# omerkurt-okt/buck-gnn

Hardware: AMD Instinct MI355X
Metric: graphs/sec (fwd+bwd) 6-layer SAGE h=512, ~5k-node meshes, batch 16, 1/2/4/8 GPU (higher is better)
Workload: dtype f32

## Files before the change

buck-gnn_amd/bgnn/_lib.py:

```python
from __future__ import annotations

import ctypes
import os
import threading

_HERE = os.path.dirname(os.path.abspath(__file__))
LIB_PATH = os.environ.get("BGNN_LIBRARY") or os.path.join(_HERE, "_lib", "libbgnn.so")
ABI_VERSION = 15

_lock = threading.Lock()
_lib = None

c_p = ctypes.c_void_p
c_i32 = ctypes.c_int32
c_i64 = ctypes.c_int64
c_f32 = ctypes.c_float
c_u64 = ctypes.c_uint64
c_sz = ctypes.c_size_t


class CsrStruct(ctypes.Structure):

    _fields_ = [
        ("rowptr", c_p),
        ("col", c_p),
        ("heavy_row", c_p),
        ("heavy_chunk0", c_p),
        ("chunk_heavy", c_p),
        ("n_rows", c_i64),
        ("nnz", c_i64),
        ("n_heavy", c_i32),
        ("n_chunks", c_i32),
        ("chunk", c_i32),
        ("ranges_all", c_i32),
        ("gsrc", c_p),
        ("gmask", c_p),
        ("gcnt", c_p),
        ("grow", c_p),
        ("n_groups", c_i64),
        ("group_rows", c_i32),
        ("_pad2", c_i32),
        ("ranges", c_p),
    ]


SIGNATURES = {
    "bgnn_abi_version": (c_i32, []),
    "bgnn_last_error_string": (ctypes.c_char_p, []),
    "bgnn_store_gather_graph": (c_i32, [c_p, c_i32, c_i64, c_i64, c_i64, c_i64, c_p, c_i64, c_p, c_p, c_p, c_p,
                                        c_p, c_p, c_p, c_p, c_p, c_p, c_p, c_p, c_p]),
    "bgnn_store_gather_rows": (c_i32, [c_p, c_i32, c_i32, c_i64, c_p, c_i64, c_p, c_p]),
    "bgnn_get_tuning": (c_i32, [c_i32]),
    "bgnn_heavy_timing": (c_i32, [c_i32]),
    "bgnn_gemm_w_tile": (c_i32, [c_i64, c_i64, c_i64]),
    "bgnn_gemm_wsplit_bytes": (c_sz, [c_i64, c_i64]),
    "bgnn_gemm_wsplit": (c_i32, [c_p, c_i32, c_i64, c_i64, c_i64, c_i64, c_p, c_i64, c_p, c_i64, c_i32, c_p]),
    "bgnn_gemm_f32_w": (c_i32, [c_i64, c_i64, c_i64, c_p, c_i64, c_p, c_i32, c_p, c_i64, c_p, c_i32, c_p, c_p, c_p,
                                c_p, c_i64, c_f32, c_u64, c_p]),
    "bgnn_heavy_timing_read": (c_i32, [c_i32, c_p, c_p]),
    "bgnn_set_tuning": (c_i32, [c_i32, c_i32]),
    "bgnn_graph_build_ws_bytes": (c_sz, [c_i64, c_i64]),
    "bgnn_graph_build": (c_i32, [c_p, c_i64, c_i64, c_p, c_p, c_p, c_p, c_p, c_p, c_sz, c_p, c_p]),
    "bgnn_index_csr_build": (c_i32, [c_p, c_i64, c_i64, c_p, c_p, c_p, c_sz, c_p, c_p]),
    "bgnn_heavy_plan_ws_bytes": (c_sz, [c_i64]),
    "bgnn_heavy_plan": (c_i32, [c_p, c_i64, c_i64, c_i32, c_p, c_p, c_p, c_p, c_p, c_sz, c_p]),
    "bgnn_spmm_fwd": (c_i32, [ctypes.POINTER(CsrStruct), c_p, c_i64, c_i32, c_i32, c_p, c_i64, c_p, c_p, c_p]),
    "bgnn_spmm_bwd": (c_i32, [ctypes.POINTER(CsrStruct), c_p, c_p, c_p, c_i64, c_i32, c_i32, c_p, c_i64, c_p, c_p,
                              c_i32, c_p]),
    "bgnn_heavy_ranges_bytes": (c_sz, [c_i32]),
    "bgnn_heavy_ranges": (c_i32, [ctypes.POINTER(CsrStruct), c_p, c_p]),
    "bgnn_range_partial_bytes": (c_sz, [c_i64, c_i32]),
    "bgnn_range_sums_finish": (c_i32, [c_p, c_i64, c_i32, ctypes.POINTER(CsrStruct), c_i32, c_p, c_i64, c_p, c_p,
                                       c_p]),
    "bgnn_bn_slots": (c_i32, [c_i64, c_i32]),
    "bgnn_bn_stats": (c_i32, [c_p, c_i64, c_i32, c_p, c_p]),
    "bgnn_bn_apply": (c_i32, [c_p, c_i64, c_i32, c_p, c_p, c_p, c_p]),
    "bgnn_bn_bwd_stats": (c_i32, [c_p, c_p, c_p, c_p, c_i64, c_i32, c_p, c_p]),
    "bgnn_bn_bwd_dx": (c_i32, [c_p, c_p, c_p, c_p, c_p, c_p, c_i64, c_i32, c_p, c_p]),
    "bgnn_spmm_bwd_add": (c_i32, [ctypes.POINTER(CsrStruct), c_p, c_p, c_p, c_i64, c_i32, c_i32, c_p, c_i64, c_p,
                                  c_i64, c_p, c_p, c_p]),
    "bgnn_spmm_bwd_max": (c_i32, [ctypes.POINTER(CsrStruct), c_p, c_p, c_i64, c_p, c_i64, c_i32, c_p, c_p, c_i64, c_p,
                                  c_i64, c_p, c_p, c_p]),
    "bgnn_spmm_max_arg_bytes": (c_sz, [c_i64, c_i32, c_i32]),
    "bgnn_sage_fwd_slots": (c_i32, [ctypes.POINTER(CsrStruct)]),
    "bgnn_group_plan": (c_i32, [c_p, c_p, c_i64, c_i32, c_i32, c_p, c_i64, c_p, c_p, c_p, c_p]),
    "bgnn_store_gather_groups": (c_i32, [c_p, c_i32, c_i32, c_i64, c_i64, c_i64, c_i64] + [c_p] * 14),
    "bgnn_sage_fwd": (c_i32, [ctypes.POINTER(CsrStruct), c_p, c_i64, c_p, c_i64, c_p, c_i32, c_i32, c_p, c_p, c_p,
                              c_p, c_p, c_i64, c_p]),
    "bgnn_bn_finalize": (c_i32, [c_p, c_i32, c_i32, c_i64, c_p, c_p, c_f32, c_f32, c_p, c_p, c_p, c_p, c_p, c_p,
                                 c_p]),
    "bgnn_bn_finalize_shifted": (c_i32, [c_p, c_i32, c_i32, c_i64, c_p, c_p, c_p, c_f32, c_f32, c_p, c_p, c_p, c_p, c_p, c_p,
                                 c_p]),
    "bgnn_bn_eval_coeffs": (c_i32, [c_i32, c_p, c_p, c_f32, c_p, c_p, c_p, c_p, c_p]),
    "bgnn_sage_apply": (c_i32, [c_p, c_p, c_p, c_p, c_i32, c_f32, c_u64, c_i64, c_i32, c_p, c_p, c_p, c_p, c_p]),
    "bgnn_sage_infer_bf16": (c_i32, [ctypes.POINTER(CsrStruct), c_p, c_i64, c_p, c_p, c_p, c_p, c_i64, c_i32, c_i32,
                                     c_p, c_i64, c_i32, c_p, c_p]),
    "bgnn_spmm_fwd_bf16": (c_i32, [ctypes.POINTER(CsrStruct), c_p, c_i64, c_i32, c_i32, c_p, c_i64, c_i32, c_p, c_p]),
    "bgnn_spmm_bwd_bf16": (c_i32, [ctypes.POINTER(CsrStruct), c_p, c_p, c_i64, c_i32, c_i32, c_p, c_i64, c_i32, c_p,
                                   c_p]),
# ... 108 lines not shown
```

buck-gnn_amd/bgnn/fused.py:

```python
from __future__ import annotations

import torch

from . import _lib
from .graph import Graph, _stream, require_cuda

GEMM_BACKEND = "hip"

PLANE_TILE = 128
Z_PLANES = False
DZ_PLANES = False
DGRAD_WT = True
FOLD_WEIGHTS_TORCH = False
DGRAD_DROPADD = True

BF16_PREP = True
ABSMAX_ITEMS = True
PERSISTENT_WPACK = True
MAX_MERGED = True
WSPLIT = True

TIMERS = None
TIMER_EVENT = None


class _timed:
    __slots__ = ("name", "ev")

    def __init__(self, name):
        self.name = name
        self.ev = None

    def __enter__(self):
        if TIMERS is not None:
            mk = TIMER_EVENT or (lambda: torch.cuda.Event(enable_timing=True))
            self.ev = (mk(), mk())
            self.ev[0].record()
        return self

    def __exit__(self, *exc):
        if self.ev is not None:
            self.ev[1].record()
            TIMERS.setdefault(self.name, []).append(self.ev)
        return False


class Planes:
    __slots__ = ("t",)

    def __init__(self, t: torch.Tensor):
        if t.dim() != 3 or not t.is_contiguous():
            raise ValueError("Planes: need a contiguous [P, rows, blk] tensor")
        self.t = t
# ... 478 lines not shown
        full = torch.empty(N + R, H, dtype=torch.float32, device=dev)
        x_next = full[:N]
        rp = torch.empty(_lib.query("bgnn_range_partial_bytes", N, H) // 4, dtype=torch.float32, device=dev)
        _lib.call("bgnn_sage_apply", o.data_ptr(), _ptr(scale), _ptr(shift), x_prev.data_ptr(), int(cfg.skip),
                  float(cfg.p), cfg.seed, N, H, x_next.data_ptr(), next_amax.data_ptr(), graph.fwd.ranges.data_ptr(),
                  rp.data_ptr(), s)
        _lib.call("bgnn_range_sums_finish", rp.data_ptr(), N, H, graph.fwd.ref(), 0, full[N:].data_ptr(), H,
                  next_amax.data_ptr(), rng.out_amax.data_ptr(), s)
        rng.holder.append(full)
        return x_next, (scale, shift, mean, invstd)
    x_next = torch.empty(N, H, dtype=torch.float32, device=dev)
    _lib.call("bgnn_sage_apply", o.data_ptr(), _ptr(scale), _ptr(shift), x_prev.data_ptr(), int(cfg.skip),
              float(cfg.p), cfg.seed, N, H, x_next.data_ptr(), next_amax.data_ptr(), None, None, s)
    return x_next, (scale, shift, mean, invstd)


def _glue_bwd_stats(g, o, scale, shift, mean, invstd, cfg: LayerConfig, g_rows=None):
    if not cfg.bn:
        return None, None, None, None
    N, H = o.shape
    dev = o.device
    s = _stream()
    rs = _lib.query("bgnn_rows_slots", N)
    part2 = torch.empty(rs, 2, H, dtype=torch.float32, device=dev)
    _lib.call("bgnn_sage_bwd_stats", g.data_ptr(), _ptr(g_rows), o.data_ptr(), scale.data_ptr(), shift.data_ptr(),
              mean.data_ptr(), invstd.data_ptr(), float(cfg.p), cfg.seed, N, H, part2.data_ptr(), s)
    sums = torch.empty(2, H, dtype=torch.float32, device=dev)
    _lib.call("bgnn_reduce_partials", part2.data_ptr(), rs, H, sums[0].data_ptr(), sums[1].data_ptr(), 0, s)
    dbeta, dgamma = sums[0], sums[1]
    if cfg.training:
        return dgamma, dbeta, sums[0], sums[1]
    z = torch.zeros(H, dtype=torch.float32, device=dev)
    return dgamma, dbeta, z, z


class SageLayerFn(torch.autograd.Function):

    @staticmethod
    def forward(ctx, x_prev, x_amax, w_l, b_l, w_r, gamma, beta, running_mean, running_var, graph: Graph,
                cfg: LayerConfig, amax=None, w_in=None, b_in=None, wprep=None, pool=None):
        dev = x_prev.device
        x_prev = x_prev.contiguous()
        H = w_l.size(0)
        N = x_prev.size(0)
        if isinstance(wprep, WPrep):
            wcat, wcat_t_pre, img_f, img_d = wprep.wcat, wprep.wcat_t, wprep, wprep
        elif wprep is not None:
            (wcat, wcat_t_pre), img_f, img_d = wprep, None, None
        else:
            wcat, wcat_t_pre, img_f, img_d = torch.cat([w_l, w_r], 0).contiguous(), None, None, None
        img_f = img_f if (img_f is not None and img_f.img_f is not None) else None
        img_d = img_d if (img_d is not None and img_d.img_d is not None) else None
        if amax is None:
            amax = torch.zeros(3, dtype=torch.float32, device=dev)
        w_amax, next_amax, dz_amax = amax[0:1], amax[1:2], amax[2:3]
        folded = w_in is not None
        if folded:
            if cfg.skip:
                raise ValueError("sage_layer: a folded input transform needs a layer without skip")
            if FOLD_WEIGHTS_TORCH:
                wf = torch.mm(wcat, w_in)
                bf = torch.mv(wcat, b_in)
            else:
                fs = cfg.famax
                fa = (fs[0:1], fs[1:2], fs[2:3]) if fs is not None else (None, None, None)
                if fs is not None:
                    absmax(wcat, fa[0], accumulate=True)
                    absmax(w_in, fa[1], accumulate=True)
                    absmax(b_in.view(1, -1), fa[2], accumulate=True)
                wf = gemm(wcat, w_in.contiguous(), trans_a=False, trans_b=False, a_amax=fa[0], b_amax=fa[1])
                bf = gemm(wcat, b_in.contiguous().view(H, 1), trans_a=False, trans_b=False, a_amax=fa[0],
                          b_amax=fa[2]).view(-1)
            absmax(wf, w_amax, accumulate=True)
            wmat = wf
        else:
            if wprep is None:
                absmax(wcat, w_amax, accumulate=True)
            wmat, bf = wcat, None
        if x_amax is None:
            x_amax = absmax(x_prev)
        planes = Z_PLANES and H % PLANE_TILE == 0 and not folded
        rng = cfg.rng
        x_full = rng.x_full if (rng is not None and rng.x_full is not None and not folded and not planes) else None
        if x_full is not None and x_full.data_ptr() != x_prev.data_ptr():
            raise RuntimeError("sage_layer: RangeRows.x_full must start at x_prev")
        xa, a_amax_g = (x_full, rng.x_amax) if x_full is not None else (x_prev, x_amax)
        M = xa.size(0)
        with _timed("gemm_fwd_fold" if folded else "gemm_fwd"):
            if planes:
                z = torch.empty(2, N, H, dtype=torch.float32, device=dev)
                gemm(x_prev, wmat, trans_a=False, trans_b=True, out=Planes(z), a_amax=x_amax, b_amax=w_amax)
                zl, zr, ldz = z[0], z[1], H
            elif (img_f is not None and not folded
                  and _lib.query("bgnn_gemm_w_tile", M, 2 * H, H) == img_f.bn_f):
                z = torch.empty(M, 2 * H, dtype=torch.float32, device=dev)
                _lib.call("bgnn_gemm_f32_w", M, 2 * H, H, xa.data_ptr(), xa.stride(0), img_f.img_f.data_ptr(),
                          img_f.bn_f, z.data_ptr(), 2 * H, None, 0, a_amax_g.data_ptr(), w_amax.data_ptr(), None, None,
                          0, 0.0, 0, _stream())
                zl, zr, ldz = z, z[:, H:], 2 * H
            else:
                z = gemm(xa, wmat, trans_a=False, trans_b=True, bias=bf, a_amax=a_amax_g, b_amax=w_amax)
                zl, zr, ldz = z, z[:, H:], 2 * H
        hagg = z[N:] if x_full is not None else None
        o = torch.empty(N, H, dtype=torch.float32, device=dev)
        nrm = torch.empty(N, dtype=torch.float32, device=dev)
        slots = _lib.query("bgnn_sage_fwd_slots", graph.fwd.ref())
        bn_part = torch.empty(slots, 2, H, dtype=torch.float32, device=dev)
        part = (torch.empty(graph.fwd.plan.n_chunks * H, dtype=torch.float32, device=dev)
                if graph.fwd.plan.n_chunks else None)
        s = _stream()
        with _timed("sage_fwd"):
            _lib.call("bgnn_sage_fwd", graph.fwd.ref(), zl.data_ptr(), ldz, zr.data_ptr(), ldz, b_l.data_ptr(), H,
                      cfg.reduce, o.data_ptr(), nrm.data_ptr(), bn_part.data_ptr(), _ptr(part), _ptr(hagg),
                      2 * H if hagg is not None else 0, s)
        del z, zl, zr, hagg
        x_next, (scale, shift, mean, invstd) = _glue_fwd(o, bn_part, slots, x_prev, gamma, beta, running_mean,
                                                         running_var, cfg, next_amax, graph)
        ctx.graph = graph
        ctx.cfg = cfg
        ctx.folded = folded
        ctx.wcat_t = wcat_t_pre
        ctx.img_d = img_d if not folded else None
        ctx.set_materialize_grads(False)
        ctx.fold = (w_in, b_in, wf) if folded else None
        ctx.save_for_backward(x_prev, o, nrm, wcat, gamma if gamma is not None else torch.empty(0, device=dev),
                              scale if scale is not None else torch.empty(0, device=dev),
                              shift if shift is not None else torch.empty(0, device=dev),
                              mean if mean is not None else torch.empty(0, device=dev),
                              invstd if invstd is not None else torch.empty(0, device=dev),
                              x_amax, w_amax, dz_amax)
        ctx.mark_non_differentiable(next_amax)
        ctx.pool = pool
        if pool is not None:
            from .ops import spmm_fwd
            pooled, _ = spmm_fwd(pool.fwd, x_next, 1, pool.num_rows)
            return x_next, next_amax, pooled
        return x_next, next_amax

    @staticmethod
    def backward(ctx, g, _g_amax, g_pool=None):
        cfg: LayerConfig = ctx.cfg
        g_rows = None
        if g_pool is not None:
            seg = ctx.pool
            gp = g_pool.contiguous() / seg.fwd.degree().clamp_min(1).to(g_pool.dtype).unsqueeze(1)
            if g is None and not cfg.skip:
                g, g_rows = gp, seg.index
            else:
                gb = gp.index_select(0, seg.index)
                g = gb if g is None else g + gb
        if g is None:
            return (None,) * 16
        x_prev, o, nrm, wcat, gamma, scale, shift, mean, invstd, x_amax, w_amax, dz_amax = ctx.saved_tensors
        graph: Graph = ctx.graph
        g = g.contiguous()
        N, H = o.shape
        planes = DZ_PLANES and H % PLANE_TILE == 0
        dev = o.device
        s = _stream()
        bn = cfg.bn
        dgamma, dbeta, sum_g2, sum_g2xhat = _glue_bwd_stats(g, o, scale, shift, mean, invstd, cfg, g_rows)
        if planes:
            dzt = torch.empty(2, N, H, dtype=torch.float32, device=dev)
            dz, dzl, dh, lddz = Planes(dzt), dzt[0], dzt[1], H
        else:
            dz = torch.empty(N, 2 * H, dtype=torch.float32, device=dev)
            dzl, dh, lddz = dz, dz[:, H:], 2 * H
        dropadd = (cfg.skip and DGRAD_DROPADD and GEMM_BACKEND == "hip" and DGRAD_WT and not planes
                   and H % 4 == 0 and _lib.query("bgnn_get_tuning", 5) == 2)
        gskip = torch.empty(N, H, dtype=torch.float32, device=dev) if (cfg.skip and not dropadd) else None
        rs = _lib.query("bgnn_rows_slots", N)
        part_db = torch.empty(rs, 2, H, dtype=torch.float32, device=dev)
        bw = graph.bwd
        rb = (cfg.rng is not None and cfg.rng.bwd and not planes and bw.ranges is not None)
        rp = (torch.empty(_lib.query("bgnn_range_partial_bytes", N, H) // 4, dtype=torch.float32, device=dev)
              if rb else None)
        _lib.call("bgnn_sage_bwd_rows", g.data_ptr(), _ptr(g_rows), o.data_ptr(), nrm.data_ptr(),
                  _ptr(scale) if bn else None, _ptr(shift) if bn else None,
                  _ptr(gamma) if (bn and gamma.numel()) else None,
                  _ptr(mean) if bn else None, _ptr(invstd) if bn else None, _ptr(sum_g2), _ptr(sum_g2xhat),
                  float(cfg.p), cfg.seed, int(cfg.skip and not dropadd), N, H, dh.data_ptr(), lddz, _ptr(gskip),
                  part_db.data_ptr(), dz_amax.data_ptr(), graph.fwd.rowptr.data_ptr() if ctx.folded else None,
                  (2 if cfg.reduce == 1 else 1) if ctx.folded else 0, _ptr(bw.ranges) if rb else None,
                  graph.fwd.rowptr.data_ptr() if (rb and cfg.reduce == 1) else None, _ptr(rp), s)
        if rb:
            _lib.call("bgnn_range_sums_finish", rp.data_ptr(), N, H, bw.ref(), 1, dzl.data_ptr(), lddz, None,
                      dz_amax.data_ptr(), s)
        db2 = torch.empty(2 if ctx.folded else 1, H, dtype=torch.float32, device=dev)
        _lib.call("bgnn_reduce_partials", part_db.data_ptr(), rs, H, db2[-1].data_ptr(),
                  db2[0].data_ptr() if ctx.folded else None, 0, s)
        db, db_zl = db2[-1], (db2[0] if ctx.folded else None)
        part = torch.empty(bw.plan.n_chunks * H, dtype=torch.float32, device=dev) if bw.plan.n_chunks else None
        with _timed("spmm_bwd"):
            _lib.call("bgnn_spmm_bwd", bw.ref(), graph.perm_t.data_ptr(), graph.fwd.rowptr.data_ptr(),
                      dh.data_ptr(), lddz, H, cfg.reduce, dzl.data_ptr(), lddz, _ptr(part),
                      dz_amax.data_ptr(), int(rb), s)
        has_affine = bn and gamma.numel() > 0
        if ctx.folded:
            w_in, b_in, wf = ctx.fold
            wf_t = wf.t().contiguous() if DGRAD_WT else wf
            with _timed("gemm_dgrad_fold"):
                dx = gemm(dz, wf_t, trans_a=False, trans_b=DGRAD_WT, a_amax=dz_amax, b_amax=w_amax)
            fs = cfg.famax
            fa = (fs[0:1], fs[1:2], fs[2:3], fs[3:4], fs[4:5]) if fs is not None else (None,) * 5
            with _timed("gemm_wgrad_fold"):
                dwf = gemm(dz, x_prev, trans_a=True, trans_b=False, a_amax=dz_amax, b_amax=x_amax,
                           c_amax=fa[3])
            dbf = db2.view(-1)
            if fs is not None:
                absmax(db2, fa[4], accumulate=True)
            if FOLD_WEIGHTS_TORCH:
                dw = torch.addmm(torch.outer(dbf, b_in), dwf, w_in.t())
                dw_in = torch.mm(wcat.t(), dwf)
                db_in = torch.mv(wcat.t(), dbf)
            else:
                dw = gemm(dwf, w_in.contiguous(), trans_a=False, trans_b=True, a_amax=fa[3],
                          b_amax=fa[1])
                dw.add_(torch.outer(dbf, b_in))
                dw_in = gemm(wcat, dwf, trans_a=True, trans_b=False, a_amax=fa[0], b_amax=fa[3])
                db_in = gemm(wcat, dbf.view(-1, 1), trans_a=True, trans_b=False, a_amax=fa[0],
                             b_amax=fa[4]).view(-1)
            return (dx, None, dw[:H], db, dw[H:], dgamma if has_affine else None, dbeta if has_affine else None,
                    None, None, None, None, None, dw_in, db_in, None, None)
        wcat_t = (ctx.wcat_t if ctx.wcat_t is not None else wcat.t().contiguous()) if DGRAD_WT else wcat
        img_d = ctx.img_d if (not planes and DGRAD_WT) else None
        if (img_d is not None and (dropadd or gskip is None)
                and _lib.query("bgnn_gemm_w_tile", N, H, 2 * H) == img_d.bn_d):
            dx = torch.empty(N, H, dtype=torch.float32, device=dev)
            with _timed("gemm_dgrad"):
                _lib.call("bgnn_gemm_f32_w", N, H, 2 * H, dz.data_ptr(), lddz, img_d.img_d.data_ptr(), img_d.bn_d,
                          dx.data_ptr(), H, None, 0, dz_amax.data_ptr(), w_amax.data_ptr(), None,
                          g.data_ptr() if dropadd else None, H, float(cfg.p) if dropadd else 0.0,
                          cfg.seed if dropadd else 0, s)
        elif dropadd:
            dx = torch.empty(N, H, dtype=torch.float32, device=dev)
            M_, K_ = N, 2 * H
            ws_bytes = _lib.query("bgnn_gemm_ws_bytes_ex", M_, H, K_, 0, 1, 0)
            ws = torch.empty(ws_bytes, dtype=torch.uint8, device=dev) if ws_bytes else None
            with _timed("gemm_dgrad"):
                _lib.call("bgnn_gemm_f32_dropadd", 0, 1, M_, H, K_, dz.data_ptr(), lddz, wcat_t.data_ptr(),
                          wcat_t.stride(0), dx.data_ptr(), H, dz_amax.data_ptr(), w_amax.data_ptr(), g.data_ptr(),
                          H, float(cfg.p), cfg.seed, _ptr(ws), ws_bytes, s)
        elif gskip is not None:
            with _timed("gemm_dgrad"):
                dx = gemm(dz, wcat_t, trans_a=False, trans_b=DGRAD_WT, out=gskip, beta=1.0, a_amax=dz_amax,
                          b_amax=w_amax)
        else:
            with _timed("gemm_dgrad"):
                dx = gemm(dz, wcat_t, trans_a=False, trans_b=DGRAD_WT, a_amax=dz_amax, b_amax=w_amax)
        with _timed("gemm_wgrad"):
            dw = gemm(dz, x_prev, trans_a=True, trans_b=False, a_amax=dz_amax, b_amax=x_amax)
        dw_l, dw_r = dw[:H], dw[H:]
        return (dx, None, dw_l, db, dw_r, dgamma if has_affine else None, dbeta if has_affine else None,
                None, None, None, None, None, None, None, None, None)


# ... 436 lines not shown
```

buck-gnn_amd/csrc/spmm.hip:

```cpp
#include <vector>

#include "common.h"
#include "gemm_common.h"
#include "seg_common.h"

namespace bgnn {

enum : int { OP_SUM = 0, OP_MEAN = 1, OP_MAX = 2, OP_MEANT = 3, OP_MAXT = 4 };
enum : int { EPI_PLAIN = 0, EPI_SAGE = 1 };

struct SegArgs {
    const int32_t* rowptr;
    const int32_t* col;
    const int32_t* heavy_row;
    const int32_t* heavy_chunk0;
    const int32_t* chunk_heavy;
    int64_t n_rows;
    int32_t n_heavy, n_chunks, chunk;
    int32_t H;
    int64_t rows_per_block;
    const float* x;     int64_t ldx;
    float* out;         int64_t ldo;
    uint8_t* arg8;
    int32_t* heavy_of;
// ... 5 lines not shown
    const uint8_t* arg8_in;
    const int32_t* heavy_of_in;
    const int32_t* arg_h_in;
    const float* zr;    int64_t ldzr;
    const float* bias;
    float* nrm;
    float* bn_partial;
    int32_t light_slots;
    int32_t nt;
    uint32_t* amax;
    const float* add;
    int64_t ld_add;
    const int32_t* gsrc;
    const uint8_t* gmask;
    const int32_t* gcnt;
    const int32_t* grow;
    int64_t n_groups;
    int32_t group_rows;
    int32_t rev;
    const int32_t* hfirst;
    const float* hagg;
    int64_t ld_hagg;
    int32_t hdone;
    int32_t ranges_all;
};

__device__ __forceinline__ bool range_row(const SegArgs& A, int32_t h) {
    return A.hfirst != nullptr && (A.hagg != nullptr || A.hdone) && A.hfirst[h] >= 0;
}

__device__ __forceinline__ void amax_flush_wave(uint32_t* amax, uint32_t m) {
    if (!amax) return;
    for (int o = 32; o > 0; o >>= 1) m = max(m, (uint32_t)__shfl_xor((int)m, o, kWave));
    if ((threadIdx.x & 63) == 0 && m) atomicMax(amax, m);
}


template <int VEC>
struct Vec {
    float f[VEC];
};

template <int VEC>
__device__ __forceinline__ Vec<VEC> ld(const float* p) {
    Vec<VEC> v;
    if constexpr (VEC == 4) {
        const float4 q = *reinterpret_cast<const float4*>(p);
        v.f[0] = q.x; v.f[1] = q.y; v.f[2] = q.z; v.f[3] = q.w;
    } else {
        v.f[0] = *p;
    }
    return v;
}

template <int VEC>
__device__ __forceinline__ void st(float* p, const Vec<VEC>& v) {
    if constexpr (VEC == 4) {
        *reinterpret_cast<float4*>(p) = make_float4(v.f[0], v.f[1], v.f[2], v.f[3]);
    } else {
        *p = v.f[0];
    }
}

template <int VEC>
__device__ __forceinline__ void ldi(const int32_t* p, int32_t (&o)[VEC]) {
    if constexpr (VEC == 4) {
        const int4 q = *reinterpret_cast<const int4*>(p);
// ... 741 lines not shown
                        *pq = s2;
                    }
                    if (lane == 0) A.nrm[r] = nr;
                }
            } else {
#pragma unroll
                for (int t = 0; t < R; ++t) {
                    const int64_t r = r0 + t;
                    const int32_t rb = __builtin_amdgcn_readlane(rp, t);
                    const int32_t deg = __builtin_amdgcn_readlane(rp, t + 1) - rb;
                    if (t >= rows || deg > chunk) continue;
                    Acc<4, NV, OP> acc;
#pragma unroll
                    for (int v = 0; v < NV; ++v)
#pragma unroll
                        for (int q = 0; q < 4; ++q) acc.a[v][q] = a[t][v][q];
                    store_plain<4, NV, OP>(A, acc, r, deg, cpos, cok, tmax);
                }
            }
        }
    }
    if constexpr (EPI == EPI_PLAIN) amax_flush_wave(A.amax, tmax);

    if constexpr (EPI == EPI_SAGE) {
        __syncthreads();
        float* dst = A.bn_partial + (int64_t)blockIdx.x * 2 * A.H;
        for (int c = threadIdx.x; c < A.H; c += 256) {
            dst[c] = (red[0][0][c] + red[1][0][c]) + (red[2][0][c] + red[3][0][c]);
            dst[A.H + c] = (red[0][1][c] + red[1][1][c]) + (red[2][1][c] + red[3][1][c]);
        }
    }
}

constexpr int kMaxLightBlocks = 1024;

static int g_seg_kernel = 0;
static int g_grp_blocks = 1024;
static int g_seg_blocks = 1024;
static int g_seg_nt = 1;
static int g_seg_u = 0;

struct Geometry {
    int vec, nv, lpr, ctiles;
};

inline int pow2ceil(int x) {
    int p = 1;
    while (p < x) p <<= 1;
    return p;
}

inline Geometry pick_geometry(int H, bool aligned16) {
    Geometry g;
    if (aligned16 && H % 4 == 0) {
        g.vec = 4;
        const int nv4 = H / 4;
        if (nv4 >= 128) { g.lpr = 64; g.nv = 2; }
        else if (nv4 > 64) { g.lpr = 64; g.nv = 2; }
        else { g.lpr = pow2ceil(nv4 < 16 ? 16 : nv4); g.nv = 1; }
        g.ctiles = (H + g.lpr * 4 * g.nv - 1) / (g.lpr * 4 * g.nv);
    } else {
        g.vec = 1;
        g.nv = 1;
        g.lpr = pow2ceil(H < 16 ? 16 : (H > 64 ? 64 : H));
        g.ctiles = (H + g.lpr - 1) / g.lpr;
    }
// ... 163 lines not shown
    A.heavy_chunk0 = c->heavy_chunk0;
    A.chunk_heavy = c->chunk_heavy;
    A.n_rows = c->n_rows;
    A.n_heavy = c->n_heavy;
    A.n_chunks = c->n_chunks;
    A.chunk = c->chunk > 0 ? c->chunk : 0x7fffffff;
    if (c->gsrc && c->gmask && c->gcnt && (c->group_rows == 4 || c->group_rows == 8)) {
        A.gsrc = c->gsrc;
        A.gmask = c->gmask;
        A.gcnt = c->gcnt;
        A.group_rows = c->group_rows;
        A.grow = c->grow;
        A.n_groups = c->grow ? c->n_groups : (c->n_rows + c->group_rows - 1) / c->group_rows;
    }
    if (c->ranges && c->n_heavy > 0) {
        A.hfirst = c->ranges + 2 + 3 * c->n_heavy;
        A.ranges_all = c->ranges_all;
    }
    return A;
}

extern int g_x6_bdma;
extern int g_h3p_nsb;
#ifdef BGNN_H3P_ABLATION
extern int g_h3p_abl;
#endif

}

using namespace bgnn;

extern "C" int bgnn_spmm_fwd(const bgnn_csr_t* csr, const float* x, int64_t ldx, int32_t H, int32_t reduce,
                             float* out, int64_t ldo, void* arg, float* partial, void* stream) {
    BGNN_REQUIRE(csr && csr->rowptr, "spmm_fwd: null csr");
    BGNN_REQUIRE(H > 0 && ldx >= H && ldo >= H, "spmm_fwd: bad H/ld");
    BGNN_REQUIRE(reduce >= 0 && reduce <= 2, "spmm_fwd: bad reduce %d", reduce);
    BGNN_REQUIRE(csr->n_chunks == 0 || partial, "spmm_fwd: partial scratch required for heavy rows");
    SegArgs A = args_from_csr(csr);
    g_heavy_dir = 0;
    A.H = H;
    A.x = x; A.ldx = ldx;
    A.out = out; A.ldo = ldo;
    if (arg) {
        BGNN_REQUIRE(csr->chunk > 0 && csr->chunk < 255,
                     "spmm_fwd(max, arg): the CSR's chunk must be in [1, 254] for the compact argmax (got %d)",
                     csr->chunk);
        const MaxArgLayout L = max_arg_layout(csr->n_rows, H);
        A.arg8 = static_cast<uint8_t*>(arg);
        A.heavy_of = reinterpret_cast<int32_t*>(static_cast<char*>(arg) + L.heavy_of);
        A.arg_h = reinterpret_cast<int32_t*>(static_cast<char*>(arg) + L.arg_h);
    }
    A.partial = partial;
    A.partial_arg = partial ? reinterpret_cast<int32_t*>(partial + (int64_t)csr->n_chunks * H) : nullptr;
    const bool al = aligned16(x) && aligned16(out) && ldx % 4 == 0 && ldo % 4 == 0 &&
                    (!partial || aligned16(partial)) && (!arg || aligned16(arg));
    const Geometry g = pick_geometry(H, al);
    hipStream_t s = as_stream(stream);
    switch (reduce) {
        case BGNN_REDUCE_SUM: return dispatch_plain<OP_SUM>(A, g, s);
        case BGNN_REDUCE_MEAN: return dispatch_plain<OP_MEAN>(A, g, s);
        default: return dispatch_plain<OP_MAX>(A, g, s);
    }
}

static int spmm_bwd_impl(const bgnn_csr_t* csr_t, const int32_t* perm_t, const int32_t* fwd_rowptr,
                         int64_t fwd_rows, const float* g, int64_t ldg, int32_t H, int32_t reduce, const void* arg,
                         const float* addend, int64_t ld_add, float* gx, int64_t ldgx, float* partial, float* amax,
                         int heavy_done, void* stream);

extern "C" int bgnn_spmm_bwd(const bgnn_csr_t* csr_t, const int32_t* perm_t, const int32_t* fwd_rowptr,
                             const float* g, int64_t ldg, int32_t H, int32_t reduce, float* gx, int64_t ldgx,
                             float* partial, float* amax, int32_t heavy_done, void* stream) {
    BGNN_REQUIRE(reduce != BGNN_REDUCE_MAX, "spmm_bwd: max aggregation takes bgnn_spmm_bwd_max");
    BGNN_REQUIRE(!heavy_done || (csr_t && csr_t->ranges), "spmm_bwd: heavy_done needs the CSR's ranges");
    return spmm_bwd_impl(csr_t, perm_t, fwd_rowptr, 0, g, ldg, H, reduce, nullptr, nullptr, 0, gx, ldgx, partial,
                         amax, heavy_done ? 1 : 0, stream);
}

extern "C" int bgnn_spmm_bwd_add(const bgnn_csr_t* csr_t, const int32_t* perm_t, const int32_t* fwd_rowptr,
                                 const float* g, int64_t ldg, int32_t H, int32_t reduce, const float* addend,
                                 int64_t ld_add, float* gx, int64_t ldgx, float* partial, float* amax, void* stream) {
    BGNN_REQUIRE(reduce != BGNN_REDUCE_MAX, "spmm_bwd_add: max aggregation takes bgnn_spmm_bwd_max");
    return spmm_bwd_impl(csr_t, perm_t, fwd_rowptr, 0, g, ldg, H, reduce, nullptr, addend, ld_add, gx, ldgx, partial,
                         amax, 0, stream);
}

// ... 128 lines not shown
                 "sage_fwd: ldzl/ldzr must be >= H and multiples of 4");
    BGNN_REQUIRE(reduce == BGNN_REDUCE_SUM || reduce == BGNN_REDUCE_MEAN, "sage_fwd: reduce must be sum/mean");
    BGNN_REQUIRE(aligned16(zl) && aligned16(zr) && aligned16(o) && aligned16(bias) && aligned16(bn_partial) &&
                     (!partial || aligned16(partial)),
                 "sage_fwd: pointers must be 16-byte aligned");
    BGNN_REQUIRE(csr->n_chunks == 0 || partial, "sage_fwd: partial scratch required for heavy rows");
    SegArgs A = args_from_csr(csr);
    g_heavy_dir = 0;
    A.H = H;
    A.x = zl; A.ldx = ldzl;
    A.zr = zr; A.ldzr = ldzr;
    A.bias = bias;
    A.out = o; A.ldo = H;
    A.nrm = nrm;
    A.bn_partial = bn_partial;
    A.partial = partial;
    if (heavy_agg) {
        BGNN_REQUIRE(csr->ranges && aligned16(heavy_agg) && ld_heavy_agg >= H && ld_heavy_agg % 4 == 0,
                     "sage_fwd: heavy_agg needs the CSR's ranges, 16-B alignment and ld >= H");
        A.hagg = heavy_agg;
        A.ld_hagg = ld_heavy_agg;
    }
    hipStream_t s = as_stream(stream);
    int64_t blocks = 0;
    if (H > 256) {
        return reduce == BGNN_REDUCE_SUM
                   ? launch_all<4, 2, 64, OP_SUM, EPI_SAGE>(A, 1, kMaxLightBlocks, s, &blocks)
                   : launch_all<4, 2, 64, OP_MEAN, EPI_SAGE>(A, 1, kMaxLightBlocks, s, &blocks);
    }
    return reduce == BGNN_REDUCE_SUM ? launch_all<4, 1, 64, OP_SUM, EPI_SAGE>(A, 1, kMaxLightBlocks, s, &blocks)
                                     : launch_all<4, 1, 64, OP_MEAN, EPI_SAGE>(A, 1, kMaxLightBlocks, s, &blocks);
}

extern "C" int bgnn_heavy_timing(int32_t enable) {
    g_heavy_on = enable != 0;
    if (g_heavy_on) g_heavy_used = 0;
    return BGNN_OK;
}

extern "C" int bgnn_heavy_timing_read(int32_t which, float* total_ms, int32_t* count) {
    BGNN_REQUIRE(total_ms && count && (which == 0 || which == 1), "heavy_timing_read: bad args");
    double t = 0.0;
    int32_t n = 0;
    for (size_t i = 0; i < g_heavy_used; ++i) {
        const HeavyEv& e = g_heavy_ev[i];
        if (e.fwd != (which == 0 ? 1 : 0)) continue;
        BGNN_HIP(hipEventSynchronize(e.b));
        float ms = 0.f;
        BGNN_HIP(hipEventElapsedTime(&ms, e.a, e.b));
        t += ms;
        ++n;
    }
    *total_ms = (float)t;
    *count = n;
    return BGNN_OK;
}

extern "C" size_t bgnn_spmm_max_arg_bytes(int64_t rows, int32_t H, int32_t n_heavy) {
    if (rows < 0 || H <= 0 || n_heavy < 0) return 0;
    return (size_t)max_arg_layout(rows, H).arg_h + (size_t)n_heavy * (size_t)H * 4;
}
```

include/bgnn.h:

```cpp
#ifndef BGNN_H
#define BGNN_H

#include <stddef.h>
#include <stdint.h>

#ifdef __cplusplus
extern "C" {
#endif

#define BGNN_ABI_VERSION 15

#define BGNN_OK 0
#define BGNN_E_ARG 1001
#define BGNN_E_WS 1002
#define BGNN_E_UNSUPPORTED 1003

#define BGNN_REDUCE_SUM 0
#define BGNN_REDUCE_MEAN 1
#define BGNN_REDUCE_MAX 2

int bgnn_abi_version(void);
const char* bgnn_last_error_string(void);

#define BGNN_TUNE_SEG_KERNEL 1
#define BGNN_TUNE_SEG_BLOCKS 2
#define BGNN_TUNE_SEG_U 3
#define BGNN_TUNE_SEG_NT 4
#define BGNN_TUNE_GEMM_MODE 5
#define BGNN_TUNE_ROWS_NT 6
#define BGNN_TUNE_GROUP_BLOCKS 7
#define BGNN_TUNE_ROWS_REV 13
#define BGNN_TUNE_GEMM_BDMA 16
int bgnn_heavy_timing(int32_t enable);
int bgnn_heavy_timing_read(int32_t which, float* total_ms, int32_t* count);
int32_t bgnn_get_tuning(int32_t knob);
int bgnn_set_tuning(int32_t knob, int32_t value);

typedef struct bgnn_csr {
    const int32_t* rowptr;
    const int32_t* col;
    const int32_t* heavy_row;
    const int32_t* heavy_chunk0;
    const int32_t* chunk_heavy;
// ... 14 lines not shown
} bgnn_csr_t;

size_t bgnn_graph_build_ws_bytes(int64_t num_edges, int64_t num_nodes);

int bgnn_graph_build(const int64_t* edge_index, int64_t num_edges, int64_t num_nodes,
                     int32_t* rowptr, int32_t* col,
                     int32_t* rowptr_t, int32_t* col_t, int32_t* perm_t,
                     void* ws, size_t ws_bytes, int32_t* dev_status, void* stream);

int bgnn_index_csr_build(const int64_t* index, int64_t n, int64_t num_rows,
                         int32_t* rowptr, int32_t* col,
                         void* ws, size_t ws_bytes, int32_t* dev_status, void* stream);

size_t bgnn_heavy_plan_ws_bytes(int64_t n_rows);
int bgnn_heavy_plan(const int32_t* rowptr, int64_t n_rows, int64_t nnz, int32_t chunk,
                    int32_t* heavy_row, int32_t* heavy_chunk0, int32_t* chunk_heavy,
                    int32_t* dev_counts, void* ws, size_t ws_bytes, void* stream);

size_t bgnn_heavy_ranges_bytes(int32_t n_heavy);
int bgnn_heavy_ranges(const bgnn_csr_t* csr, int32_t* ranges, void* stream);

size_t bgnn_range_partial_bytes(int64_t n_rows, int32_t H);
int bgnn_range_sums_finish(const float* range_partial, int64_t n_rows, int32_t H, const bgnn_csr_t* csr,
                           int32_t mode, float* out, int64_t ldo, const float* amax_floor, float* amax,
                           void* stream);

int bgnn_group_plan(const int32_t* rowptr, const int32_t* col, int64_t n_rows, int32_t chunk,
                    int32_t group_rows, const int32_t* grow, int64_t n_groups,
                    int32_t* gsrc, uint8_t* gmask, int32_t* gcnt, void* stream);

int bgnn_spmm_fwd(const bgnn_csr_t* csr, const float* x, int64_t ldx, int32_t H,
                  int32_t reduce, float* out, int64_t ldo, void* arg,
                  float* partial, void* stream);
size_t bgnn_spmm_max_arg_bytes(int64_t n_rows, int32_t H, int32_t n_heavy);

int bgnn_spmm_bwd(const bgnn_csr_t* csr_t, const int32_t* perm_t, const int32_t* fwd_rowptr,
                  const float* g, int64_t ldg, int32_t H, int32_t reduce,
                  float* gx, int64_t ldgx, float* partial, float* amax, int32_t heavy_done, void* stream);
int bgnn_spmm_bwd_add(const bgnn_csr_t* csr_t, const int32_t* perm_t, const int32_t* fwd_rowptr,
                      const float* g, int64_t ldg, int32_t H, int32_t reduce,
                      const float* addend, int64_t ld_add, float* gx, int64_t ldgx, float* partial,
                      float* amax, void* stream);
int bgnn_spmm_bwd_max(const bgnn_csr_t* csr_t, const int32_t* perm_t, const int32_t* fwd_rowptr,
                      int64_t fwd_rows, const float* g, int64_t ldg, int32_t H, const void* arg,
                      const float* addend, int64_t ld_add, float* gx, int64_t ldgx, float* partial,
                      float* amax, void* stream);

int32_t bgnn_sage_fwd_slots(const bgnn_csr_t* csr);
int bgnn_sage_fwd(const bgnn_csr_t* csr, const float* zl, int64_t ldzl, const float* zr, int64_t ldzr,
                  const float* bias, int32_t H, int32_t reduce, float* o, float* nrm,
                  float* bn_partial, float* partial, const float* heavy_agg, int64_t ld_heavy_agg,
                  void* stream);

int bgnn_bn_finalize(const float* bn_partial, int32_t n_slots, int32_t H, int64_t count,
                     const float* gamma, const float* beta, float eps, float momentum,
                     float* running_mean, float* running_var,
                     float* mean, float* invstd, float* scale, float* shift, void* stream);
int bgnn_bn_eval_coeffs(int32_t H, const float* gamma, const float* beta, float eps,
                        const float* running_mean, const float* running_var,
                        float* scale, float* shift, void* stream);

int bgnn_sage_apply(const float* o, const float* scale, const float* shift,
                    const float* x_prev, int32_t skip, float p, uint64_t seed,
                    int64_t n_rows, int32_t H, float* x_next, float* amax,
                    const int32_t* ranges, float* range_partial, void* stream);

int bgnn_sage_infer_bf16(const bgnn_csr_t* csr, const void* z, int64_t ldz, const float* bias,
                         const float* scale, const float* shift, const void* x_prev, int64_t ldx,
                         int32_t H, int32_t reduce, void* out, int64_t ldo, int32_t out_f32,
                         float* partial, void* stream);

int bgnn_spmm_fwd_bf16(const bgnn_csr_t* csr, const void* x, int64_t ldx, int32_t H, int32_t reduce,
                       void* out, int64_t ldo, int32_t out_f32, float* partial, void* stream);
int bgnn_spmm_bwd_bf16(const bgnn_csr_t* csr_t, const int32_t* fwd_rowptr, const void* g, int64_t ldg,
                       int32_t H, int32_t reduce, void* gx, int64_t ldgx, int32_t out_f32,
                       float* partial, void* stream);

int32_t bgnn_rows_slots(int64_t n_rows);
int bgnn_sage_bwd_stats(const float* g, const int64_t* g_rows, const float* o, const float* scale,
                        const float* shift,
                        const float* mean, const float* invstd, float p, uint64_t seed,
                        int64_t n_rows, int32_t H, float* partial2, void* stream);

int32_t bgnn_linear_bwd_prep_slots(void);
int bgnn_linear_bwd_prep(const float* g, const float* y, int64_t N, int32_t C, float* g_out,
// ... 158 lines not shown
```

Measured before the change: 2077.

## Add aggregate-first path for folded input SAGE layer and skip redundant amax atomics

Adds an optional path for the folded first layer. It aggregates the narrow input features over the graph first, then runs one GEMM on the concatenated [agg, h] against the folded weights, followed by a new row kernel that applies bias, degree-weighted bias, L2 norm and BN partial sums. The backward pass mirrors this with a dgrad GEMM into a K-wide buffer, a transposed SpMM with addend, and a paired wgrad. The intent is to do the sparse aggregation at width K<H instead of H. The path is gated by FOLD_AGG_FIRST=False and a tuning query, so it is off by default. Separately, the wave amax flush now reads the current value first and skips the atomicMax when it would not raise it, which does run by default.

```diff
diff --git a/buck-gnn_amd/bgnn/_lib.py b/buck-gnn_amd/bgnn/_lib.py
--- a/buck-gnn_amd/bgnn/_lib.py
+++ b/buck-gnn_amd/bgnn/_lib.py
@@ -6,7 +6,7 @@
 
 _HERE = os.path.dirname(os.path.abspath(__file__))
 LIB_PATH = os.environ.get("BGNN_LIBRARY") or os.path.join(_HERE, "_lib", "libbgnn.so")
-ABI_VERSION = 15
+ABI_VERSION = 16
 
 _lock = threading.Lock()
 _lib = None
@@ -65,6 +65,10 @@
     "bgnn_heavy_plan_ws_bytes": (c_sz, [c_i64]),
     "bgnn_heavy_plan": (c_i32, [c_p, c_i64, c_i64, c_i32, c_p, c_p, c_p, c_p, c_p, c_sz, c_p]),
     "bgnn_spmm_fwd": (c_i32, [ctypes.POINTER(CsrStruct), c_p, c_i64, c_i32, c_i32, c_p, c_i64, c_p, c_p, c_p]),
+    "bgnn_spmm_fwd_amax": (c_i32, [ctypes.POINTER(CsrStruct), c_p, c_i64, c_i32, c_i32, c_p, c_i64, c_p, c_p, c_p,
+                                   c_p]),
+    "bgnn_sage_rows_fwd_slots": (c_i32, [c_i64]),
+    "bgnn_sage_rows_fwd": (c_i32, [c_p, c_i64, c_p, c_p, c_p, c_i32, c_i64, c_i32, c_p, c_p, c_p, c_p]),
     "bgnn_spmm_bwd": (c_i32, [ctypes.POINTER(CsrStruct), c_p, c_p, c_p, c_i64, c_i32, c_i32, c_p, c_i64, c_p, c_p,
                               c_i32, c_p]),
     "bgnn_heavy_ranges_bytes": (c_sz, [c_i32]),
diff --git a/buck-gnn_amd/bgnn/fused.py b/buck-gnn_amd/bgnn/fused.py
--- a/buck-gnn_amd/bgnn/fused.py
+++ b/buck-gnn_amd/bgnn/fused.py
@@ -19,6 +19,7 @@
 PERSISTENT_WPACK = True
 MAX_MERGED = True
 WSPLIT = True
+FOLD_AGG_FIRST = False
 
 TIMERS = None
 TIMER_EVENT = None
@@ -563,6 +564,32 @@
         return dgamma, dbeta, sums[0], sums[1]
     z = torch.zeros(H, dtype=torch.float32, device=dev)
     return dgamma, dbeta, z, z
+
+
+def _fold_aggfirst_fwd(ctx, h, h_amax, wf, bf, b_l, w_amax, graph: Graph, cfg: LayerConfig, H: int):
+    N, K = h.shape
+    dev = h.device
+    s = _stream()
+    fw = graph.fwd
+    agg = torch.empty(N, K, dtype=torch.float32, device=dev)
+    a_amax = h_amax.clone()
+    part = torch.empty(fw.plan.n_chunks * K, dtype=torch.float32, device=dev) if fw.plan.n_chunks else None
+    with _timed("agg_fwd_fold"):
+        _lib.call("bgnn_spmm_fwd_amax", fw.ref(), h.data_ptr(), h.stride(0), K, cfg.reduce, agg.data_ptr(), K, None,
+                  _ptr(part), a_amax.data_ptr(), s)
+    wk = torch.cat([wf[:H], wf[H:]], 1)
+    with _timed("gemm_fwd_fold"):
+        y = gemm(Pair(agg, h), wk, trans_a=False, trans_b=True, a_amax=a_amax, b_amax=w_amax)
+    c = bf[H:] + b_l
+    o = torch.empty(N, H, dtype=torch.float32, device=dev)
+    nrm = torch.empty(N, dtype=torch.float32, device=dev)
+    slots = _lib.query("bgnn_sage_rows_fwd_slots", N)
+    bn_part = torch.empty(slots, 2, H, dtype=torch.float32, device=dev)
+    with _timed("rows_fwd_fold"):
+        _lib.call("bgnn_sage_rows_fwd", y.data_ptr(), y.stride(0), c.data_ptr(), bf.data_ptr(), fw.rowptr.data_ptr(),
+                  2 if cfg.reduce == 1 else 1, N, H, o.data_ptr(), nrm.data_ptr(), bn_part.data_ptr(), s)
+    ctx.aggfirst = (agg, a_amax, wk)
+    return o, nrm, bn_part, slots
 
 
 class SageLayerFn(torch.autograd.Function):
@@ -610,6 +637,17 @@
             wmat, bf = wcat, None
         if x_amax is None:
             x_amax = absmax(x_prev)
+        K_in = x_prev.size(1)
+        rng_bwd = (cfg.rng is not None and cfg.rng.bwd and graph.bwd.ranges is not None
+                   and not (DZ_PLANES and H % PLANE_TILE == 0))
+        agg_first = (folded and FOLD_AGG_FIRST and cfg.reduce in (0, 1) and GEMM_BACKEND == "hip" and not rng_bwd
+                     and K_in % 32 == 0 and K_in < H and _lib.query("bgnn_get_tuning", 5) == 2)
+        ctx.aggfirst = None
+        if agg_first:
+            o, nrm, bn_part, slots = _fold_aggfirst_fwd(ctx, x_prev, x_amax, wf, bf, b_l, w_amax, graph, cfg, H)
+            return SageLayerFn._finish_fwd(ctx, x_prev, o, nrm, bn_part, slots, wcat, wcat_t_pre, None, gamma, beta,
+                                           running_mean, running_var, graph, cfg, folded, (w_in, b_in, wf), x_amax,
+                                           w_amax, next_amax, dz_amax, pool)
         planes = Z_PLANES and H % PLANE_TILE == 0 and not folded
         rng = cfg.rng
         x_full = rng.x_full if (rng is not None and rng.x_full is not None and not folded and not planes) else None
@@ -645,6 +683,14 @@
                       cfg.reduce, o.data_ptr(), nrm.data_ptr(), bn_part.data_ptr(), _ptr(part), _ptr(hagg),
                       2 * H if hagg is not None else 0, s)
         del z, zl, zr, hagg
+        return SageLayerFn._finish_fwd(ctx, x_prev, o, nrm, bn_part, slots, wcat, wcat_t_pre, img_d, gamma, beta,
+                                       running_mean, running_var, graph, cfg, folded,
+                                       (w_in, b_in, wf) if folded else None, x_amax, w_amax, next_amax, dz_amax, pool)
+
+    @staticmethod
+    def _finish_fwd(ctx, x_prev, o, nrm, bn_part, slots, wcat, wcat_t_pre, img_d, gamma, beta, running_mean,
+                    running_var, graph, cfg, folded, fold, x_amax, w_amax, next_amax, dz_amax, pool):
+        dev = x_prev.device
         x_next, (scale, shift, mean, invstd) = _glue_fwd(o, bn_part, slots, x_prev, gamma, beta, running_mean,
                                                          running_var, cfg, next_amax, graph)
         ctx.graph = graph
@@ -653,7 +699,7 @@
         ctx.wcat_t = wcat_t_pre
         ctx.img_d = img_d if not folded else None
         ctx.set_materialize_grads(False)
-        ctx.fold = (w_in, b_in, wf) if folded else None
+        ctx.fold = fold
         ctx.save_for_backward(x_prev, o, nrm, wcat, gamma if gamma is not None else torch.empty(0, device=dev),
                               scale if scale is not None else torch.empty(0, device=dev),
                               shift if shift is not None else torch.empty(0, device=dev),
@@ -667,6 +713,25 @@
             pooled, _ = spmm_fwd(pool.fwd, x_next, 1, pool.num_rows)
             return x_next, next_amax, pooled
         return x_next, next_amax
+
+    @staticmethod
+    def _fold_weight_grads(dx, dwf, db2, db, wcat, w_in, b_in, fa, H, dgamma, dbeta, has_affine):
+        dbf = db2.view(-1)
+        if fa[4] is not None:
+            absmax(db2, fa[4], accumulate=True)
+        if FOLD_WEIGHTS_TORCH:
+            dw = torch.addmm(torch.outer(dbf, b_in), dwf, w_in.t())
+            dw_in = torch.mm(wcat.t(), dwf)
+            db_in = torch.mv(wcat.t(), dbf)
+        else:
+            dw = gemm(dwf, w_in.contiguous(), trans_a=False, trans_b=True, a_amax=fa[3],
+                      b_amax=fa[1])
+            dw.add_(torch.outer(dbf, b_in))
+            dw_in = gemm(wcat, dwf, trans_a=True, trans_b=False, a_amax=fa[0], b_amax=fa[3])
+            db_in = gemm(wcat, dbf.view(-1, 1), trans_a=True, trans_b=False, a_amax=fa[0],
+                         b_amax=fa[4]).view(-1)
+        return (dx, None, dw[:H], db, dw[H:], dgamma if has_affine else None, dbeta if has_affine else None,
+                None, None, None, None, None, dw_in, db_in, None, None)
 
     @staticmethod
     def backward(ctx, g, _g_amax, g_pool=None):
@@ -686,12 +751,16 @@
         graph: Graph = ctx.graph
         g = g.contiguous()
         N, H = o.shape
-        planes = DZ_PLANES and H % PLANE_TILE == 0
+        aggfirst = ctx.aggfirst
+        planes = DZ_PLANES and H % PLANE_TILE == 0 and aggfirst is None
         dev = o.device
         s = _stream()
         bn = cfg.bn
         dgamma, dbeta, sum_g2, sum_g2xhat = _glue_bwd_stats(g, o, scale, shift, mean, invstd, cfg, g_rows)
-        if planes:
+        if aggfirst is not None:
+            dz = dh = torch.empty(N, H, dtype=torch.float32, device=dev)
+            dzl, lddz = None, H
+        elif planes:
             dzt = torch.empty(2, N, H, dtype=torch.float32, device=dev)
             dz, dzl, dh, lddz = Planes(dzt), dzt[0], dzt[1], H
         else:
@@ -703,7 +772,7 @@
         rs = _lib.query("bgnn_rows_slots", N)
         part_db = torch.empty(rs, 2, H, dtype=torch.float32, device=dev)
         bw = graph.bwd
-        rb = (cfg.rng is not None and cfg.rng.bwd and not planes and bw.ranges is not None)
+        rb = (cfg.rng is not None and cfg.rng.bwd and not planes and bw.ranges is not None and aggfirst is None)
         rp = (torch.empty(_lib.query("bgnn_range_partial_bytes", N, H) // 4, dtype=torch.float32, device=dev)
               if rb else None)
         _lib.call("bgnn_sage_bwd_rows", g.data_ptr(), _ptr(g_rows), o.data_ptr(), nrm.data_ptr(),
@@ -721,12 +790,39 @@
         _lib.call("bgnn_reduce_partials", part_db.data_ptr(), rs, H, db2[-1].data_ptr(),
                   db2[0].data_ptr() if ctx.folded else None, 0, s)
         db, db_zl = db2[-1], (db2[0] if ctx.folded else None)
+        has_affine = bn and gamma.numel() > 0
+        if aggfirst is not None:
+            agg, a_amax, wk = aggfirst
+            w_in, b_in, wf = ctx.fold
+            K = x_prev.size(1)
+            wk_t = wk.t().contiguous() if DGRAD_WT else wk
+            with _timed("gemm_dgrad_fold"):
+                dcat = gemm(dh, wk_t, trans_a=False, trans_b=DGRAD_WT, a_amax=dz_amax, b_amax=w_amax)
+            dx = torch.empty(N, K, dtype=torch.float32, device=dev)
+            part = torch.empty(bw.plan.n_chunks * K, dtype=torch.float32, device=dev) if bw.plan.n_chunks else None
+            with _timed("spmm_bwd_fold"):
+                _lib.call("bgnn_spmm_bwd_add", bw.ref(), graph.perm_t.data_ptr(), graph.fwd.rowptr.data_ptr(),
+                          dcat.data_ptr(), 2 * K, K, cfg.reduce, dcat[:, K:].data_ptr(), 2 * K, dx.data_ptr(), K,
+                          _ptr(part), None, s)
+            fs = cfg.famax
+            fa = (fs[0:1], fs[1:2], fs[2:3], fs[3:4], fs[4:5]) if fs is not None else (None,) * 5
+            with _timed("gemm_wgrad_fold"):
+                if K % PLANE_TILE == 0:
+                    dwk_t = gemm(Pair(agg, x_prev), dh, trans_a=True, trans_b=False, a_amax=a_amax, b_amax=dz_amax,
+                                 c_amax=fa[3])
+                else:
+                    dwk_t = torch.empty(2 * K, H, dtype=torch.float32, device=dev)
+                    for half, a_half in ((dwk_t[:K], agg), (dwk_t[K:], x_prev)):
+                        gemm(a_half, dh, trans_a=True, trans_b=False, out=half, a_amax=a_amax, b_amax=dz_amax,
+                             c_amax=fa[3])
+            dwf = torch.cat([dwk_t[:K].t(), dwk_t[K:].t()], 0)
+            return SageLayerFn._fold_weight_grads(dx, dwf, db2, db, wcat, w_in, b_in, fa, H, dgamma, dbeta,
+                                                  has_affine)
         part = torch.empty(bw.plan.n_chunks * H, dtype=torch.float32, device=dev) if bw.plan.n_chunks else None
         with _timed("spmm_bwd"):
             _lib.call("bgnn_spmm_bwd", bw.ref(), graph.perm_t.data_ptr(), graph.fwd.rowptr.data_ptr(),
                       dh.data_ptr(), lddz, H, cfg.reduce, dzl.data_ptr(), lddz, _ptr(part),
                       dz_amax.data_ptr(), int(rb), s)
-        has_affine = bn and gamma.numel() > 0
         if ctx.folded:
             w_in, b_in, wf = ctx.fold
             wf_t = wf.t().contiguous() if DGRAD_WT else wf
@@ -737,22 +833,8 @@
             with _timed("gemm_wgrad_fold"):
                 dwf = gemm(dz, x_prev, trans_a=True, trans_b=False, a_amax=dz_amax, b_amax=x_amax,
                            c_amax=fa[3])
-            dbf = db2.view(-1)
-            if fs is not None:
-                absmax(db2, fa[4], accumulate=True)
-            if FOLD_WEIGHTS_TORCH:
-                dw = torch.addmm(torch.outer(dbf, b_in), dwf, w_in.t())
-                dw_in = torch.mm(wcat.t(), dwf)
-                db_in = torch.mv(wcat.t(), dbf)
-            else:
-                dw = gemm(dwf, w_in.contiguous(), trans_a=False, trans_b=True, a_amax=fa[3],
-                          b_amax=fa[1])
-                dw.add_(torch.outer(dbf, b_in))
-                dw_in = gemm(wcat, dwf, trans_a=True, trans_b=False, a_amax=fa[0], b_amax=fa[3])
-                db_in = gemm(wcat, dbf.view(-1, 1), trans_a=True, trans_b=False, a_amax=fa[0],
-                             b_amax=fa[4]).view(-1)
-            return (dx, None, dw[:H], db, dw[H:], dgamma if has_affine else None, dbeta if has_affine else None,
-                    None, None, None, None, None, dw_in, db_in, None, None)
+            return SageLayerFn._fold_weight_grads(dx, dwf, db2, db, wcat, w_in, b_in, fa, H, dgamma, dbeta,
+                                                  has_affine)
         wcat_t = (ctx.wcat_t if ctx.wcat_t is not None else wcat.t().contiguous()) if DGRAD_WT else wcat
         img_d = ctx.img_d if (not planes and DGRAD_WT) else None
         if (img_d is not None and (dropadd or gskip is None)
diff --git a/buck-gnn_amd/csrc/spmm.hip b/buck-gnn_amd/csrc/spmm.hip
--- a/buck-gnn_amd/csrc/spmm.hip
+++ b/buck-gnn_amd/csrc/spmm.hip
@@ -61,7 +61,8 @@
 __device__ __forceinline__ void amax_flush_wave(uint32_t* amax, uint32_t m) {
     if (!amax) return;
     for (int o = 32; o > 0; o >>= 1) m = max(m, (uint32_t)__shfl_xor((int)m, o, kWave));
-    if ((threadIdx.x & 63) == 0 && m) atomicMax(amax, m);
+    if ((threadIdx.x & 63) == 0 && m > __hip_atomic_load(amax, __ATOMIC_RELAXED, __HIP_MEMORY_SCOPE_AGENT))
+        atomicMax(amax, m);
 }
 
 
@@ -869,6 +870,113 @@
     }
 }
 
+struct RowsArgs {
+    const float* y;     int64_t ldy;
+    const float* c;
+    const float* v;
+    const int32_t* rowptr;
+    int32_t w_mode;
+    int64_t n_rows;
+    int32_t H;
+    float* o;
+    float* nrm;
+    float* bn_partial;
+    int32_t nt;
+};
+
+template <int NV>
+__global__ __launch_bounds__(256) void k_rows_sage(RowsArgs P) {
+    constexpr int RB = 4;
+    const int lane = threadIdx.x & 63;
+    const int wave = __builtin_amdgcn_readfirstlane(threadIdx.x >> 6);
+    const Sweep sw = sweep_rows(P.n_rows, wave);
+    int cpos[NV];
+    bool cok[NV];
+    lane_cols<4, NV, 64>(0, lane, P.H, cpos, cok);
+    float cb[NV][4], vb[NV][4], bs[NV][4], bq[NV][4];
+#pragma unroll
+    for (int v = 0; v < NV; ++v) {
+        const Vec<4> cc = ld<4>(P.c + (cok[v] ? cpos[v] : 0));
+        Vec<4> vv = cc;
+        if (P.w_mode) vv = ld<4>(P.v + (cok[v] ? cpos[v] : 0));
+#pragma unroll
+        for (int q = 0; q < 4; ++q) {
+            cb[v][q] = cc.f[q];
+            vb[v][q] = P.w_mode ? vv.f[q] : 0.f;
+            bs[v][q] = bq[v][q] = 0.f;
+        }
+    }
+    for (int t0 = 0; t0 < sw.T; t0 += 64) {
+        const int nrow = min(64, sw.T - t0);
+        float wl = 0.f;
+        if (P.w_mode && lane < nrow) {
+            const int64_t rl = sw.first + (int64_t)sw.W * (t0 + lane);
+            const int32_t d = P.rowptr[rl + 1] - P.rowptr[rl];
+            wl = (P.w_mode == 1) ? (float)d : (d > 0 ? 1.f : 0.f);
+        }
+        for (int k = 0; k < nrow; k += RB) {
+            Vec<4> yv[RB][NV];
+#pragma unroll
+            for (int q = 0; q < RB; ++q) {
+                const int kk = (k + q < nrow) ? k + q : k;
+                const int64_t r = sw.first + (int64_t)sw.W * (t0 + kk);
+#pragma unroll
+                for (int v = 0; v < NV; ++v) {
+                    const float* p = P.y + r * P.ldy + (cok[v] ? cpos[v] : 0);
+                    yv[q][v] = P.nt ? ld_nt(p) : ld<4>(p);
+                }
+            }
+#pragma unroll
+            for (int q = 0; q < RB; ++q) {
+                if (k + q >= nrow) break;
+                const int64_t r = sw.first + (int64_t)sw.W * (t0 + k + q);
+                const float w = __int_as_float(__builtin_amdgcn_readlane(__float_as_int(wl), k + q));
+                float h[NV][4];
+                float ss = 0.f;
+#pragma unroll
+                for (int v = 0; v < NV; ++v)
+#pragma unroll
+                    for (int e = 0; e < 4; ++e) {
+                        h[v][e] = cok[v] ? __fadd_rn(__fadd_rn(yv[q][v].f[e], __fmul_rn(w, vb[v][e])), cb[v][e]) : 0.f;
+                        ss = fmaf(h[v][e], h[v][e], ss);
+                    }
+                ss = group_sum(ss, kWave);
+                const float n = sqrtf(ss);
+                const float d = fmaxf(n, 1e-12f);
+#pragma unroll
+                for (int v = 0; v < NV; ++v) {
+                    if (!cok[v]) continue;
+                    Vec<4> ov;
+#pragma unroll
+                    for (int e = 0; e < 4; ++e) {
+                        ov.f[e] = h[v][e] / d;
+                        bs[v][e] += ov.f[e];
+                        bq[v][e] += ov.f[e] * ov.f[e];
+                    }
+                    if (P.nt) st_nt(P.o + r * P.H + cpos[v], ov);
+                    else st<4>(P.o + r * P.H + cpos[v], ov);
+                }
+                if (lane == 0) P.nrm[r] = n;
+            }
+        }
+    }
+    __shared__ __attribute__((aligned(16))) float red[4][2][512];
+#pragma unroll
+    for (int v = 0; v < NV; ++v)
+        if (cok[v])
+#pragma unroll
+            for (int e = 0; e < 4; ++e) {
+                red[wave][0][cpos[v] + e] = bs[v][e];
+                red[wave][1][cpos[v] + e] = bq[v][e];
+            }
+    __syncthreads();
+    float* dst = P.bn_partial + (int64_t)blockIdx.x * 2 * P.H;
+    for (int col = threadIdx.x; col < P.H; col += 256) {
+        dst[col] = (red[0][0][col] + red[1][0][col]) + (red[2][0][col] + red[3][0][col]);
+        dst[P.H + col] = (red[0][1][col] + red[1][1][col]) + (red[2][1][col] + red[3][1][col]);
+    }
+}
+
 constexpr int kMaxLightBlocks = 1024;
 
 static int g_seg_kernel = 0;
@@ -1098,6 +1206,11 @@
 
 extern "C" int bgnn_spmm_fwd(const bgnn_csr_t* csr, const float* x, int64_t ldx, int32_t H, int32_t reduce,
                              float* out, int64_t ldo, void* arg, float* partial, void* stream) {
+    return bgnn_spmm_fwd_amax(csr, x, ldx, H, reduce, out, ldo, arg, partial, nullptr, stream);
+}
+
+extern "C" int bgnn_spmm_fwd_amax(const bgnn_csr_t* csr, const float* x, int64_t ldx, int32_t H, int32_t reduce,
+                                  float* out, int64_t ldo, void* arg, float* partial, float* amax, void* stream) {
     BGNN_REQUIRE(csr && csr->rowptr, "spmm_fwd: null csr");
     BGNN_REQUIRE(H > 0 && ldx >= H && ldo >= H, "spmm_fwd: bad H/ld");
     BGNN_REQUIRE(reduce >= 0 && reduce <= 2, "spmm_fwd: bad reduce %d", reduce);
@@ -1118,6 +1231,7 @@
     }
     A.partial = partial;
     A.partial_arg = partial ? reinterpret_cast<int32_t*>(partial + (int64_t)csr->n_chunks * H) : nullptr;
+    A.amax = reinterpret_cast<uint32_t*>(amax);
     const bool al = aligned16(x) && aligned16(out) && ldx % 4 == 0 && ldo % 4 == 0 &&
                     (!partial || aligned16(partial)) && (!arg || aligned16(arg));
     const Geometry g = pick_geometry(H, al);
@@ -1312,6 +1426,28 @@
                                      : launch_all<4, 1, 64, OP_MEAN, EPI_SAGE>(A, 1, kMaxLightBlocks, s, &blocks);
 }
 
+extern "C" int32_t bgnn_sage_rows_fwd_slots(int64_t n_rows) {
+    return n_rows < 0 ? -1 : (int32_t)sweep_grid(n_rows);
+}
+
+extern "C" int bgnn_sage_rows_fwd(const float* y, int64_t ldy, const float* c, const float* v, const int32_t* rowptr,
+                                  int32_t w_mode, int64_t n_rows, int32_t H, float* o, float* nrm, float* bn_partial,
+                                  void* stream) {
+    BGNN_REQUIRE(y && c && o && nrm && bn_partial && n_rows >= 0, "sage_rows_fwd: null argument");
+    BGNN_REQUIRE(H > 0 && H <= 512 && H % 4 == 0, "sage_rows_fwd: H=%d unsupported (need H%%4==0, H<=512)", H);
+    BGNN_REQUIRE(ldy >= H && ldy % 4 == 0, "sage_rows_fwd: ldy must be >= H and a multiple of 4");
+    BGNN_REQUIRE(w_mode >= 0 && w_mode <= 2 && (w_mode == 0 || (rowptr && v)), "sage_rows_fwd: bad row weights");
+    BGNN_REQUIRE(aligned16(y) && aligned16(c) && aligned16(o) && aligned16(bn_partial) && (!v || aligned16(v)),
+                 "sage_rows_fwd: pointers must be 16-byte aligned");
+    RowsArgs P{y, ldy, c, v, rowptr, w_mode, n_rows, H, o, nrm, bn_partial, g_seg_nt};
+    hipStream_t s = as_stream(stream);
+    const dim3 gr((unsigned)sweep_grid(n_rows));
+    if (H > 256) hipLaunchKernelGGL((k_rows_sage<2>), gr, dim3(256), 0, s, P);
+    else hipLaunchKernelGGL((k_rows_sage<1>), gr, dim3(256), 0, s, P);
+    BGNN_CHECK_LAUNCH();
+    return BGNN_OK;
+}
+
 extern "C" int bgnn_heavy_timing(int32_t enable) {
     g_heavy_on = enable != 0;
     if (g_heavy_on) g_heavy_used = 0;
diff --git a/include/bgnn.h b/include/bgnn.h
--- a/include/bgnn.h
+++ b/include/bgnn.h
@@ -8,7 +8,7 @@
 extern "C" {
 #endif
 
-#define BGNN_ABI_VERSION 15
+#define BGNN_ABI_VERSION 16
 
 #define BGNN_OK 0
 #define BGNN_E_ARG 1001
@@ -89,6 +89,9 @@
 int bgnn_spmm_fwd(const bgnn_csr_t* csr, const float* x, int64_t ldx, int32_t H,
                   int32_t reduce, float* out, int64_t ldo, void* arg,
                   float* partial, void* stream);
+int bgnn_spmm_fwd_amax(const bgnn_csr_t* csr, const float* x, int64_t ldx, int32_t H,
+                       int32_t reduce, float* out, int64_t ldo, void* arg,
+                       float* partial, float* amax, void* stream);
 size_t bgnn_spmm_max_arg_bytes(int64_t n_rows, int32_t H, int32_t n_heavy);
 
 int bgnn_spmm_bwd(const bgnn_csr_t* csr_t, const int32_t* perm_t, const int32_t* fwd_rowptr,
@@ -108,6 +111,11 @@
                   const float* bias, int32_t H, int32_t reduce, float* o, float* nrm,
                   float* bn_partial, float* partial, const float* heavy_agg, int64_t ld_heavy_agg,
                   void* stream);
+
+int32_t bgnn_sage_rows_fwd_slots(int64_t n_rows);
+int bgnn_sage_rows_fwd(const float* y, int64_t ldy, const float* c, const float* v, const int32_t* rowptr,
+                       int32_t w_mode, int64_t n_rows, int32_t H, float* o, float* nrm, float* bn_partial,
+                       void* stream);
 
 int bgnn_bn_finalize(const float* bn_partial, int32_t n_slots, int32_t H, int64_t count,
                      const float* gamma, const float* beta, float eps, float momentum,
```

Measured after the change: 2088 (median of 6 runs). No clear change (+0.5%).
